# gbbin/DDP-practice

Measured on AMD Instinct MI355X. Metric: images/sec (whole node) + 3-epoch wall-clock, MNIST ConvNet at 1/2/4/8 MI355X, higher is better.
Workload: dtype bf16; 1 GPU; model=ConvNet (2x[Conv5x5-BN-ReLU-MaxPool2] + Linear(1568,10), 29,034 params), global_batch=32, parallelism=dp1, per_rank_batch=32, impl=native (fused HIP kernels, C++ reducer/communicator), sync_bn=False, amp=autocast bf16 + GradScaler, optimizer=SGD(lr=1e-4), hipgraph=True, steps_per_graph=16, comm=none (1 rank), grad_avg=none (1 rank)

## Files before the change

ddp_practice_amd/csrc/kernels/conv5x5.h:

```cpp
#pragma once
#include "convblock_bn.h"

namespace dpa {
namespace cb {

template <int I> struct SH;
template <> struct SH<0> { static constexpr int CIN = 1, COUT = 16, H = 28, W = 28, SPLIT = 4, WROWS = 28; };
template <> struct SH<1> { static constexpr int CIN = 16, COUT = 32, H = 14, W = 14, SPLIT = 2, WROWS = 14; };

__host__ __device__ constexpr int conv5x5_win_rows(int H, int W, int nsplit, bool even) {
  const int HW = H * W, MT = (HW + 15) / 16;
  int mx = 0;
  for (int sp = 0; sp < nsplit; ++sp) {
    const int p0 = 16 * (MT * sp / nsplit), p1e = 16 * (MT * (sp + 1) / nsplit), p1 = p1e < HW ? p1e : HW;
    if (p1 <= p0) return 0;
    int lo = p0 / W - 2, hi = (p1 - 1) / W + 2;
    lo = lo < 0 ? 0 : lo;
    hi = hi > H - 1 ? H - 1 : hi;
    if (even) {
      lo &= ~1;
      hi |= 1;
    }
    mx = hi - lo + 1 > mx ? hi - lo + 1 : mx;
  }
  return mx;
}

template <typename T>
struct BwdEpi {
  const uint8_t* idx;
  const T* xh;
  float* bslab;
};

constexpr int W2F_ROWS = 32, W2F_PITCH = 424;
constexpr int W2D_ROWS = 16, W2D_PITCH = 808;
constexpr int W2F_LEN = W2F_ROWS * W2F_PITCH, W2D_LEN = W2D_ROWS * W2D_PITCH;
template <typename T>
struct WPack {
  const float* w2 = nullptr;
  T* fwd = nullptr;
  T* dgrad = nullptr;
};
template <typename T>
__device__ __forceinline__ void pack_w2(const WPack<T>& pk) {
  const int total = W2F_LEN + W2D_LEN;
  for (int e = blockIdx.x * blockDim.x + threadIdx.x; e < total; e += gridDim.x * blockDim.x) {
    if (e < W2F_LEN) {
      const int co = e / W2F_PITCH, k = e % W2F_PITCH;
      const float v = k < 400 ? pk.w2[(co * 16 + (k & 15)) * 25 + (k >> 4)] : 0.f;
      pk.fwd[e] = Cvt<T>::from_f(v);
    } else {
      const int e2 = e - W2F_LEN;
      const int ci = e2 / W2D_PITCH, k = e2 % W2D_PITCH;
      const float v = k < 800 ? pk.w2[((k & 31) * 16 + ci) * 25 + (24 - (k >> 5))] : 0.f;
      pk.dgrad[e2] = Cvt<T>::from_f(v);
    }
  }
}

struct GatherIn {
  const uint8_t* imgs = nullptr;
  const int64_t* labels = nullptr;
  const int64_t* order = nullptr;
  long long order_len = 0;
  int* ctr = nullptr;
  int64_t* lab_out = nullptr;
  float scale = 1.f, shift = 0.f;
  int nimg = 0;
};

template <typename T, int CIN, int H, int W>
__host__ __device__ constexpr size_t conv5x5_img_bytes() {
  return ((sizeof(T) * (size_t)(H + 4) * (W + 4) * CIN) + 15) / 16 * 16;
}
template <typename T, int CIN, int COUT, int H, int W>
__host__ __device__ constexpr size_t conv5x5_dyn_bytes() {
  return conv5x5_img_bytes<T, CIN, H, W>() + sizeof(T) * (size_t)COUT * (ceil_to(25 * CIN, 32) + 8);
}

template <typename T, int CIN, int COUT, int H, int W, int MODE, int PRO = 0, int EPI = 0, int WPK = 0,
          bool DYN = false, int WR = H>
__device__ __forceinline__ void
conv5x5_body(const T* __restrict__ x, const float* __restrict__ w, const float* __restrict__ bias,
             T* __restrict__ y, float* __restrict__ fslab, float* __restrict__ fstats,
             const float* __restrict__ shift, int nsplit, const PoolIn<T>& pin, const BwdIn<T>& bin,
             const BwdEpi<T>& epi, const T* __restrict__ wpk, const WPack<T>& pk, const int bid,
             const GatherIn& gin = GatherIn{}) {
  static_assert(CIN == 1 || CIN % 8 == 0, "CIN must be 1 or a multiple of 8");
  static_assert(COUT % 16 == 0, "COUT must be a multiple of 16");
  static_assert((H * W) % 4 == 0, "H*W must be a multiple of 4");
  static_assert(PRO != 2 || MODE == 2, "PRO 2 is a data-grad prologue");
  static_assert(PRO != 3 || (CIN == 1 && MODE != 2), "PRO 3 gathers single-channel input images");
  static_assert(EPI == 0 || MODE == 2, "EPI 1 is a data-grad epilogue");
  constexpr int NCH = CIN >= 8 ? CIN / 8 : 1;
  constexpr int HP = H + 4, WPD = W + 4;
  constexpr int K = 25 * CIN;
  constexpr int KP = ceil_to(K, 32);
  constexpr int KS = KP / 32;
  constexpr int KPW = KP + 8;
  constexpr int NT = COUT / 16;
  constexpr int HW = H * W;
  constexpr int MT = (HW + 15) / 16;
  typedef MM<T> mm;

  T* img;
  T* wl;
  if constexpr (DYN) {
    img = reinterpret_cast<T*>(dpa_dyn_lds);
    wl = reinterpret_cast<T*>(dpa_dyn_lds + conv5x5_img_bytes<T, CIN, H, W>());
  } else {
    __shared__ __attribute__((aligned(16))) T img_s[HP * WPD * CIN];
    __shared__ __attribute__((aligned(16))) T wl_s[COUT * KPW];
    img = img_s;
    wl = wl_s;
  }
  constexpr int PPB = NCH <= 16 ? 16 / NCH : 1;
  auto imo = [](int px, int c) -> int {
    if constexpr (NCH <= 1) {
      return px * CIN + c;
    } else {
      return px * CIN + ((((c >> 3) ^ ((px / PPB) & (NCH - 1)))) << 3) + (c & 7);
    }
  };
  __shared__ float lstat[(NTHR / 64) * 2 * COUT];

  const int tid = threadIdx.x;
  const int b = bid / nsplit;
  DPA_STAMP(0);
  const int sp = bid % nsplit;
  const T* xb = x + (size_t)b * CIN * HW;
  const int mt0 = (MT * sp) / nsplit, mt1 = (MT * (sp + 1)) / nsplit;
  constexpr bool WIN = WR < H;
  static_assert(!WIN || PRO == 1 || PRO == 2, "row windows: the BN prologues' staging passes");
  static_assert(WR >= 1 && (PRO != 2 || WR % 2 == 0 || !WIN), "PRO 2 stages whole 2x2 windows");
  constexpr int SR = WIN ? WR : H;
  const int p_lo = mt0 * 16, p_hi = min(mt1 * 16, HW);
  int r_lo = 0, r_n = H, z_lo = 0, z_n = HP;
  if constexpr (WIN) {
    const int oh_lo = p_lo / W, oh_hi = (p_hi - 1) / W;
    r_lo = max(oh_lo - 2, 0);
    int r_hi = min(oh_hi + 2, H - 1);
    if constexpr (PRO == 2) {
      r_lo &= ~1;
      r_hi |= 1;
    }
    r_n = r_hi - r_lo + 1;
    z_lo = oh_lo;
    z_n = oh_hi + 5 - oh_lo;
  }
  float pre_bias[NT], pre_shift[NT];
#pragma unroll
  for (int nt = 0; nt < NT; ++nt) {
    const int co = nt * 16 + (tid & 15);
    pre_bias[nt] = (MODE == 2) ? 0.f : bias[co];
    pre_shift[nt] = (MODE == 0) ? shift[co] : 0.f;
  }

  const T zero = Cvt<T>::from_f(0.f);
  constexpr int WN16 = WPK == 1 ? COUT * KPW * (int)sizeof(T) / 16 : 1;
  constexpr int WIT = (WN16 + NTHR - 1) / NTHR;
  auto load_wpk = [&]() {
    if constexpr (WPK == 1) {
      static_assert((COUT * KPW * sizeof(T)) % 16 == 0, "packed weight tile must be whole 16-B chunks");
      static_assert(COUT * KPW == (MODE == 2 ? W2D_LEN : W2F_LEN), "pre-packed weights exist for layer 2 only");
      typedef __attribute__((address_space(3))) void* lds_ptr_t;
      const uint4* src = reinterpret_cast<const uint4*>(wpk);
      uint4* dstl = reinterpret_cast<uint4*>(wl);
      const int wv0 = (tid >> 6) * 64, ln = tid & 63;
#pragma unroll
      for (int i = 0; i < WIT; ++i) {
        const int c0 = i * NTHR + wv0;
        if (c0 + ln < WN16)
          __builtin_amdgcn_global_load_lds(src + c0 + ln, (lds_ptr_t)(dstl + c0), 16, 0, 0);
      }
    }
  };
  if constexpr (WPK == 1) {
    if constexpr (PRO == 0 || PRO == 3) load_wpk();
  } else {
    if constexpr (KP > K) {
      for (int e = tid; e < COUT * (KP - K); e += NTHR) wl[(e / (KP - K)) * KPW + K + e % (KP - K)] = zero;
    }
    constexpr int KO = 25 * (MODE == 2 ? COUT : CIN);
    stage_f32<COUT * K>(w, [&](int e, float v) {
      const int o = e / KO, rem = e % KO;
      const int i = rem / 25, tap = rem % 25;
      if (MODE == 2)
        wl[i * KPW + (24 - tap) * CIN + o] = Cvt<T>::from_f(v);
      else
        wl[o * KPW + tap * CIN + i] = Cvt<T>::from_f(v);
    });
  }
  if constexpr (WPK == 2) pack_w2<T>(pk);
  DPA_STAMP(1);
  if constexpr ((CIN * sizeof(T)) % 16 == 0) {
    constexpr int G = CIN * (int)sizeof(T) / 16;
    uint4* img4 = reinterpret_cast<uint4*>(img);
    if constexpr (WIN) {
      uint4* row4 = img4 + z_lo * WPD * G;
      for (int e = tid; e < z_n * WPD * G; e += NTHR) {
        const int px = e / G, hp = z_lo + px / WPD, wp = px % WPD;
        if (hp < 2 || hp >= H + 2 || wp < 2 || wp >= W + 2) row4[e] = make_uint4(0u, 0u, 0u, 0u);
      }
    } else {
      for (int e = tid; e < HP * WPD * G; e += NTHR) {
        const int px = e / G, hp = px / WPD, wp = px % WPD;
        if (hp < 2 || hp >= H + 2 || wp < 2 || wp >= W + 2) img4[e] = make_uint4(0u, 0u, 0u, 0u);
      }
    }
  } else {
    static_assert(!WIN, "row windows: whole 16-B channel groups per pixel");
    for (int e = tid; e < HP * WPD * CIN; e += NTHR) {
      const int hp = e / (WPD * CIN), rem = e % (WPD * CIN);
      const int wp = rem / CIN;
      if (hp < 2 || hp >= H + 2 || wp < 2 || wp >= W + 2) img[e] = zero;
    }
  }
  constexpr int EPIX = EPI ? MT * 16 : 1;
  __shared__ uint8_t eidx[EPI ? COUT * EPIX : 1];
  __shared__ T exh[EPI ? COUT * EPIX : 1];
  const int ep0 = mt0 * 16, enp = min(mt1 * 16, HW) - ep0;
  constexpr int EIT = EPI ? (COUT * EPIX + NTHR - 1) / NTHR : 1;
  uint8_t ei[EIT];
  T ex[EIT];
  auto load_epi = [&]() {
    if constexpr (EPI == 1) {
#pragma unroll
      for (int i = 0; i < EIT; ++i) {
        const int e = tid + i * NTHR;
        const int ec = e < COUT * enp ? e : 0;
        const int co = ec / enp, pp = ec % enp;
        const size_t o = ((size_t)b * COUT + co) * HW + ep0 + pp;
        ei[i] = epi.idx[o];
        ex[i] = epi.xh[o];
      }
    }
  };
  auto store_epi = [&]() {
    if constexpr (EPI == 1) {
#pragma unroll
      for (int i = 0; i < EIT; ++i) {
        const int e = tid + i * NTHR;
        if (e < COUT * enp) {
          const int co = e / enp, pp = e % enp;
          eidx[co * EPIX + pp] = ei[i];
          exh[co * EPIX + pp] = ex[i];
        }
      }
    }
  };
  if constexpr (PRO != 2) {
    load_epi();
    store_epi();
  }
  DPA_STAMP(2);
  constexpr int DQ = PRO != 1 ? 1
                     : (CIN % 8 == 0 && sizeof(T) == 2) ? 8 * ((CIN / 8 * SR * W + NTHR - 1) / NTHR)
                                                          : (CIN * SR * W + NTHR - 1) / NTHR;
  int dq_e[DQ];
  T dq_p[DQ], dq_x[DQ];
  uint8_t dq_i[DQ];
#pragma unroll
  for (int d = 0; d < DQ; ++d) dq_e[d] = -1;
  if constexpr (PRO == 0) {
    stage_chw<T, CIN, H, W>(xb, [&](int ci, int h, int ww, T a, T bb) {
      img[imo((h + 2) * WPD + (ww + 2), ci)] = a;
      img[imo((h + 2) * WPD + (ww + 3), ci)] = bb;
    });
  } else if constexpr (PRO == 3) {
    static_assert(HW % 4 == 0 && W % 4 == 0, "4-pixel groups stay inside a row");
    constexpr int G4 = HW / 4, GIT = (G4 + NTHR - 1) / NTHR;
    const int step = __builtin_amdgcn_readfirstlane(*reinterpret_cast<volatile int*>(gin.ctr));
    long long pos = (long long)step * gin.nimg + b;
    pos = pos < gin.order_len ? pos : gin.order_len - 1;
    const int64_t src = gin.order[pos];
    const uint32_t* s4 = reinterpret_cast<const uint32_t*>(gin.imgs + src * HW);
    uint32_t v4[GIT];
#pragma unroll
    for (int i = 0; i < GIT; ++i)
      if (tid + i * NTHR < G4) v4[i] = s4[tid + i * NTHR];
    if (sp == 0 && tid == 0) gin.lab_out[b] = gin.labels[src];
    T* xo = const_cast<T*>(xb);
#pragma unroll
    for (int i = 0; i < GIT; ++i) {
      const int g = tid + i * NTHR;
      if (g < G4) {
        const int h = (4 * g) / W, ww = (4 * g) % W;
        T px[4];
#pragma unroll
        for (int k = 0; k < 4; ++k) {
          px[k] = Cvt<T>::from_f((float)((v4[i] >> (8 * k)) & 0xffu) * gin.scale + gin.shift);
          img[imo((h + 2) * WPD + (ww + k + 2), 0)] = px[k];
        }
        if (sp == 0) {
#pragma unroll
          for (int k = 0; k < 4; ++k) xo[4 * g + k] = px[k];
        }
      }
    }
    if (tid == 0) {
      const int arrived = __hip_atomic_fetch_add(&gin.ctr[1], 1, __ATOMIC_RELAXED, __HIP_MEMORY_SCOPE_AGENT);
      if (arrived == gin.nimg * nsplit - 1) {
        __hip_atomic_store(&gin.ctr[1], 0, __ATOMIC_RELAXED, __HIP_MEMORY_SCOPE_AGENT);
        __hip_atomic_store(&gin.ctr[0], step + 1, __ATOMIC_RELAXED, __HIP_MEMORY_SCOPE_AGENT);
      }
    }
  } else if constexpr (PRO == 1) {
    __shared__ float sc_s[CIN], beta_s[CIN], mean_s[CIN], istd_s[CIN];
    __shared__ float part[NTHR];
    typedef typename Pair2<T>::type P;
    constexpr int RP = SR * W;
    const T* yb = pin.y + (size_t)b * CIN * 4 * HW;
    const bool wr = pin.p_out != nullptr;
    if constexpr (CIN % 8 == 0 && sizeof(T) == 2) {
      constexpr int NO = CIN / 8, NPI = NO * RP, IT8 = (NPI + NTHR - 1) / NTHR;
      P top[IT8][8], bot[IT8][8];
      auto ld8 = [&](int i, int o, int ho, int wo) {
#pragma unroll
        for (int j = 0; j < 8; ++j) {
          const P* src = reinterpret_cast<const P*>(yb + ((size_t)(8 * o + j) * 2 * H + 2 * ho) * 2 * W + 2 * wo);
          top[i][j] = src[0];
          bot[i][j] = src[W];
        }
      };
#pragma unroll
      for (int i = 0; i < IT8; ++i) {
        const int e8 = tid + i * NTHR;
        if constexpr (WIN) {
          const int ec = min(e8, NPI - 1);
          ld8(i, ec / RP, min(r_lo + (ec % RP) / W, H - 1), ec % W);
        } else if (e8 < NPI) {
          ld8(i, e8 / RP, (e8 % RP) / W, e8 % W);
        }
      }
      load_wpk();
      bn_finalize<CIN>(pin.bn, sc_s, beta_s, mean_s, istd_s, part, bid);
      DPA_STAMP(3);
#pragma unroll
      for (int i = 0; i < IT8; ++i) {
        const int e8 = tid + i * NTHR;
        const int o = e8 / RP, hl = (e8 % RP) / W, ho = r_lo + hl, wo = e8 % W;
        if (e8 < NPI && (!WIN || hl < r_n)) {
          const int pix = ho * W + wo;
          const bool own = wr && pix >= p_lo && pix < p_hi;
          unsigned pk[4];
#pragma unroll
          for (int j = 0; j < 8; ++j) {
            const int ci = 8 * o + j;
            float best, xh;
            int bi;
            bn_relu_max4x<T>(top[i][j], bot[i][j], sc_s[ci], beta_s[ci], mean_s[ci], istd_s[ci], best, bi, xh);
            const T pvj = Cvt<T>::from_f(best);
            const unsigned bits = __builtin_bit_cast(unsigned short, pvj);
            if (j & 1) pk[j >> 1] |= bits << 16; else pk[j >> 1] = bits;
            const int e = ci * HW + pix;
            const int d = i * 8 + j;
            dq_e[d] = own ? e : -1;
            dq_p[d] = pvj;
            dq_i[d] = (uint8_t)(bi | (best > 0.f ? IDX_RELU : 0));
            dq_x[d] = Cvt<T>::from_f(xh);
          }
          *reinterpret_cast<uint4*>(&img[imo((ho + 2) * WPD + (wo + 2), 8 * o)]) = make_uint4(pk[0], pk[1], pk[2], pk[3]);
        }
      }
    } else {
      constexpr int NPS = CIN * RP, IT = (NPS + NTHR - 1) / NTHR;
      P top[IT], bot[IT];
      auto ld1 = [&](int i, int ci, int ho, int wo) {
        const P* src = reinterpret_cast<const P*>(yb + ((size_t)ci * 2 * H + 2 * ho) * 2 * W + 2 * wo);
        top[i] = src[0];
        bot[i] = src[W];
      };
#pragma unroll
      for (int i = 0; i < IT; ++i) {
        const int e = tid + i * NTHR;
        if constexpr (WIN) {
          const int ec = min(e, NPS - 1);
          ld1(i, ec / RP, min(r_lo + (ec % RP) / W, H - 1), ec % W);
        } else if (e < NPS) {
          ld1(i, e / RP, (e % RP) / W, e % W);
        }
      }
      load_wpk();
      bn_finalize<CIN>(pin.bn, sc_s, beta_s, mean_s, istd_s, part, bid);
      DPA_STAMP(3);
#pragma unroll
      for (int i = 0; i < IT; ++i) {
        const int e = tid + i * NTHR;
        const int ci = e / RP, hl = (e % RP) / W, ho = r_lo + hl, wo = e % W;
        if (e < NPS && (!WIN || hl < r_n)) {
          const int pix = ho * W + wo;
          float best, xh;
          int bi;
          bn_relu_max4x<T>(top[i], bot[i], sc_s[ci], beta_s[ci], mean_s[ci], istd_s[ci], best, bi, xh);
          const T pv = Cvt<T>::from_f(best);
          img[imo((ho + 2) * WPD + (wo + 2), ci)] = pv;
          dq_e[i] = wr && pix >= p_lo && pix < p_hi ? ci * HW + pix : -1;
          dq_p[i] = pv;
          dq_i[i] = (uint8_t)(bi | (best > 0.f ? IDX_RELU : 0));
          dq_x[i] = Cvt<T>::from_f(xh);
        }
      }
    }
  } else {
    __shared__ float coef[5 * CIN], sums[2 * CIN];
    __shared__ float part[NTHR];
    if constexpr (CIN % 8 == 0 && sizeof(T) == 2) {
      BnBwdStage8<T, CIN, H, W, NTHR, SR> st;
      st.load(bin, b, r_lo);
      DPA_STAMP(8);
      load_wpk();
      bn_bwd_coef<CIN, T>(bin, coef, part, sums, bid);
      load_epi();
      DPA_STAMP(3);
      st.emit(coef, [&](int h, int ww, int c0, uint4 q00, uint4 q01, uint4 q10, uint4 q11) {
        if (WIN && h >= r_n) return;
        const int hp = r_lo + h + 2;
        *reinterpret_cast<uint4*>(&img[imo(hp * WPD + (ww + 2), c0)]) = q00;
        *reinterpret_cast<uint4*>(&img[imo(hp * WPD + (ww + 3), c0)]) = q01;
        *reinterpret_cast<uint4*>(&img[imo((hp + 1) * WPD + (ww + 2), c0)]) = q10;
        *reinterpret_cast<uint4*>(&img[imo((hp + 1) * WPD + (ww + 3), c0)]) = q11;
      });
    } else {
      BnBwdStage<T, CIN, H, W, NTHR, SR> st;
      st.load(bin, b, r_lo);
      DPA_STAMP(8);
      load_wpk();
      bn_bwd_coef<CIN, T>(bin, coef, part, sums, bid);
      load_epi();
      DPA_STAMP(3);
      st.emit(coef, [&](int c, int h, int ww, T v00, T v01, T v10, T v11) {
        if (WIN && h >= r_n) return;
        const int hp = r_lo + h + 2;
        img[imo(hp * WPD + (ww + 2), c)] = v00;
        img[imo(hp * WPD + (ww + 3), c)] = v01;
        img[imo((hp + 1) * WPD + (ww + 2), c)] = v10;
        img[imo((hp + 1) * WPD + (ww + 3), c)] = v11;
      });
    }
    store_epi();
  }
  DPA_STAMP(4);
  __syncthreads();
  DPA_STAMP(5);
  if constexpr (PRO == 1) {
    constexpr int NPO = CIN * HW;
#pragma unroll
    for (int d = 0; d < DQ; ++d)
      if (dq_e[d] >= 0) {
        const size_t o = (size_t)b * NPO + dq_e[d];
        pin.p_out[o] = dq_p[d];
        pin.idx_out[o] = dq_i[d];
        pin.xh_out[o] = dq_x[d];
      }
  }

  const int lane = tid & 63, wv = tid >> 6;
  const int r = lane & 15, q = lane >> 4;

  float s1[NT], s2[NT];
#pragma unroll
  for (int nt = 0; nt < NT; ++nt) s1[nt] = s2[nt] = 0.f;

  for (int mt = mt0 + wv; mt < mt1; mt += NTHR / 64) {
    const int m = mt * 16 + r;
    const int mm_ = m < HW ? m : HW - 1;
    const int oh = mm_ / W, ow = mm_ % W;
    f32x4 acc[NT];
#pragma unroll
    for (int nt = 0; nt < NT; ++nt) acc[nt] = f32x4{0.f, 0.f, 0.f, 0.f};
#pragma unroll
    for (int s = 0; s < KS; ++s) {
      typename mm::frag a;
      if constexpr (CIN == 1) {
#pragma unroll
        for (int j = 0; j < 8; ++j) {
          const int tap = 32 * s + 8 * q + j;
          float v = 0.f;
          if (tap < 25) v = Cvt<T>::to_f(img[(oh + tap / 5) * WPD + ow + tap % 5]);
          a[j] = mm::cv(v);
        }
      } else {
        const int kb = 32 * s + 8 * q;
        int tap = kb / CIN;
        const int ci0 = kb % CIN;
        tap = tap < 25 ? tap : 24;
        a = mm::ld(&img[imo((oh + tap / 5) * WPD + ow + tap % 5, ci0)]);
      }
#pragma unroll
      for (int nt = 0; nt < NT; ++nt) {
        const typename mm::frag bf = mm::ld(&wl[(nt * 16 + r) * KPW + 32 * s + 8 * q]);
        acc[nt] = mm::mma(a, bf, acc[nt]);
      }
    }
    const int pix0 = mt * 16 + 4 * q;
    if (pix0 < HW) {
#pragma unroll
      for (int nt = 0; nt < NT; ++nt) {
        const int co = nt * 16 + r;
        const float bs = pre_bias[nt];
        T* dst = y + ((size_t)b * COUT + co) * HW + pix0;
        const float sh = pre_shift[nt];
#pragma unroll
        for (int i = 0; i < 4; ++i) {
          const float v = acc[nt][i] + bs;
          dst[i] = Cvt<T>::from_f(v);
          if (MODE == 0) {
            const float d = rnd_t<T>(v) - sh;
            s1[nt] += d;
            s2[nt] += d * d;
          }
          if (EPI == 1) {
            const int le = co * EPIX + pix0 - mt0 * 16 + i;
            const float g = (eidx[le] & IDX_RELU) ? rnd_t<T>(v) : 0.f;
            s1[nt] += g;
            s2[nt] += g * Cvt<T>::to_f(exh[le]);
          }
        }
      }
    }
  }
  DPA_STAMP(6);
  if constexpr (MODE == 0 || EPI == 1) {
#pragma unroll
    for (int nt = 0; nt < NT; ++nt) {
      const float a1 = xor32_sum(xor16_sum(s1[nt])), a2 = xor32_sum(xor16_sum(s2[nt]));
      if (q == 0) {
        lstat[wv * 2 * COUT + nt * 16 + r] = a1;
        lstat[wv * 2 * COUT + COUT + nt * 16 + r] = a2;
      }
    }
    __syncthreads();
    float* row = (MODE == 0 ? fslab + (size_t)bid * fslab_row(COUT)
                            : epi.bslab + (size_t)bid * 2 * COUT);
    if (tid < 2 * COUT) {
      float t = 0.f;
#pragma unroll
      for (int w2 = 0; w2 < NTHR / 64; ++w2) t += lstat[w2 * 2 * COUT + tid];
      row[tid] = t;
    }
    if constexpr (MODE == 0) {
      if (tid == 0) {
        const int p0 = mt0 * 16, p1 = min(mt1 * 16, HW);
        row[2 * COUT] = (float)(p1 - p0);
      }
      if (bid == 0 && tid < COUT) fstats[2 * COUT + 1 + tid] = shift[tid];
    }
  }
  DPA_STAMP(7);
}

template <typename T, int CIN, int COUT, int H, int W, int MODE, int PRO = 0, int EPI = 0, int WPK = 0, int WR = H>
__global__ void __launch_bounds__(NTHR)
conv5x5_kernel(const T* __restrict__ x, const float* __restrict__ w, const float* __restrict__ bias,
               T* __restrict__ y, float* __restrict__ fslab, float* __restrict__ fstats,
               const float* __restrict__ shift, int nsplit, PoolIn<T> pin = PoolIn<T>{},
               BwdIn<T> bin = BwdIn<T>{}, BwdEpi<T> epi = BwdEpi<T>{}, const T* __restrict__ wpk = nullptr,
               WPack<T> pk = WPack<T>{}, GatherIn gin = GatherIn{}) {
  conv5x5_body<T, CIN, COUT, H, W, MODE, PRO, EPI, WPK, false, WR>(x, w, bias, y, fslab, fstats, shift, nsplit, pin,
                                                                   bin, epi, wpk, pk, (int)blockIdx.x, gin);
}

}
}
```

ddp_practice_amd/csrc/kernels/convnet_fused.hip:

```cpp
#include <type_traits>

#include "conv5x5.h"
#include "conv5x5_wgrad.h"
#include "comm/xgmi.h"

namespace dpa {
namespace cnf {

using cb::BNParams;
using cb::bn_finalize;
using cb::bn_relu_max4x;
using cb::BwdEpi;
using cb::BwdIn;
using cb::IDX_POS;
using cb::IDX_RELU;
using cb::Pair2;
using cb::PoolIn;
using cb::with_t;

constexpr int HF = 256;
constexpr int NTHR_HB = 256;

template <typename T, int C, int H, int W, int NMAX>
__global__ void __launch_bounds__(HF)
// ... 177 lines not shown
}

typedef std::shared_ptr<xgmi::XgmiComm> XcPtr;
static xgmi::XSite site_of(const XcPtr& xc, int s) { return xc ? xc->site(s) : xgmi::XSite{}; }

int64_t fwd2_split(bool fp32) { return fp32 ? cb::kFwd2SplitT<float> : cb::kFwd2SplitT<__half>; }

template <int NSPLIT, bool EVEN>
constexpr int conv2_wr() {
  constexpr int need = cb::conv5x5_win_rows(14, 14, NSPLIT, EVEN);
  static_assert(need > 0, "conv2: more workgroups per image than 16-pixel tiles");
  return need < 14 ? need : 14;
}
static void conv2_row_window(int wr, int nsplit, bool even, const char* what) {
  const int need = cb::conv5x5_win_rows(14, 14, nsplit, even);
  TORCH_CHECK(need > 0 && (wr >= 14 || need <= wr), what, ": a split in ", nsplit, " stages up to ", need,
              " rows, the kernel's window holds ", wr);
}
template <typename T>
constexpr int kFwd2WR = conv2_wr<cb::kFwd2SplitT<T>, false>();

void conv2_fwd(at::Tensor y1, c10::optional<at::Tensor> fslab1, at::Tensor fstats1, at::Tensor g1, at::Tensor b1,
               at::Tensor rm1, at::Tensor rv1, at::Tensor nbt1, double momentum, double eps, bool train, at::Tensor w2,
               at::Tensor bias2, at::Tensor y2, c10::optional<at::Tensor> fslab2, at::Tensor fstats2, at::Tensor rm2,
               c10::optional<at::Tensor> p1_out, c10::optional<at::Tensor> idx1_out,
               c10::optional<at::Tensor> xh1_out, at::Tensor wpk, XcPtr xc) {
  DPA_CHECK_INPUT(y1); DPA_CHECK_INPUT(w2); DPA_CHECK_INPUT(y2); DPA_CHECK_INPUT(wpk);
  TORCH_CHECK(wpk.numel() == cb::W2F_LEN && wpk.scalar_type() == y1.scalar_type(), "packed conv2 weights");
  const int B = (int)y1.size(0);
  TORCH_CHECK(y1.size(1) == 16 && y1.size(2) == 28 && y1.size(3) == 28 && w2.size(0) == 32 && w2.size(1) == 16,
              "fused conv2 expects the ConvNet shapes");
  TORCH_CHECK(y2.scalar_type() == y1.scalar_type());
  TORCH_CHECK(p1_out.has_value() == idx1_out.has_value() && p1_out.has_value() == xh1_out.has_value());
  if (p1_out.has_value())
    TORCH_CHECK(p1_out->numel() == (int64_t)B * 16 * 196 && idx1_out->numel() == p1_out->numel() &&
                xh1_out->numel() == p1_out->numel());
  const int ns = fwd2_split(y1.scalar_type() == at::kFloat);
  if (train) TORCH_CHECK(fslab2.has_value() && fslab2->numel() == (int64_t)B * ns * cb::fslab_row(32));
  if (B == 0) return;
  BNParams bp = bn_params(fslab1, fstats1, g1, b1, rm1, rv1, nbt1, momentum, eps, train, 16);
  if (train) {
    bp.xs = site_of(xc, xgmi::kSiteFwd1);
    xgmi::set_site_grid(bp.xs, B * ns, "conv2_fwd");
  }
  hipStream_t stream = cur_stream();
  with_t(dt_of(y1), [&](auto tag) {
    typedef decltype(tag) T;
    PoolIn<T> pin{dptr<T>(y1), bp, p1_out.has_value() ? dptr<T>(*p1_out) : nullptr,
                  idx1_out.has_value() ? idx1_out->data_ptr<uint8_t>() : nullptr,
                  xh1_out.has_value() ? dptr<T>(*xh1_out) : nullptr};
    constexpr int WR = kFwd2WR<T>;
    conv2_row_window(WR, ns, false, "conv2_fwd");
    if (train)
      hipLaunchKernelGGL((cb::conv5x5_kernel<T, 16, 32, 14, 14, 0, 1, 0, 1, WR>), dim3(B * ns), dim3(cb::NTHR), 0,
                         stream, nullptr, nullptr, bias2.data_ptr<float>(), dptr<T>(y2), fslab2->data_ptr<float>(),
                         fstats2.data_ptr<float>(), rm2.data_ptr<float>(), ns, pin, BwdIn<T>{}, BwdEpi<T>{},
                         dptr<T>(wpk), cb::WPack<T>{});
    else
      hipLaunchKernelGGL((cb::conv5x5_kernel<T, 16, 32, 14, 14, 1, 1, 0, 1, WR>), dim3(B * ns), dim3(cb::NTHR), 0,
                         stream, nullptr, nullptr, bias2.data_ptr<float>(), dptr<T>(y2), nullptr, nullptr, nullptr,
                         ns, pin, BwdIn<T>{}, BwdEpi<T>{}, dptr<T>(wpk), cb::WPack<T>{});
  });
  DPA_CHECK_LAUNCH();
}

void head_fwd(at::Tensor y2, c10::optional<at::Tensor> fslab2, at::Tensor fstats2, at::Tensor g2, at::Tensor b2,
              at::Tensor rm2, at::Tensor rv2, at::Tensor nbt2, double momentum, double eps, bool train, at::Tensor wfc,
              at::Tensor bfc, at::Tensor logits, c10::optional<at::Tensor> p2_out, c10::optional<at::Tensor> idx2_out,
              c10::optional<at::Tensor> xh2_out, XcPtr xc) {
  DPA_CHECK_INPUT(y2); DPA_CHECK_INPUT(wfc); DPA_CHECK_INPUT(logits);
  const int B = (int)y2.size(0), N = (int)wfc.size(0);
  TORCH_CHECK(y2.size(1) == 32 && y2.size(2) == 14 && y2.size(3) == 14 && wfc.size(1) == 32 * 49,
              "fused head expects the ConvNet shapes");
  TORCH_CHECK(N >= 1 && N <= 64, "fused head supports up to 64 classes");
  TORCH_CHECK(logits.numel() == (int64_t)B * N && logits.scalar_type() == y2.scalar_type());
  TORCH_CHECK(p2_out.has_value() == idx2_out.has_value() && p2_out.has_value() == xh2_out.has_value());
  if (p2_out.has_value())
    TORCH_CHECK(p2_out->numel() == (int64_t)B * 1568 && idx2_out->numel() == p2_out->numel() &&
                xh2_out->numel() == p2_out->numel());
  if (B == 0) return;
  BNParams bp = bn_params(fslab2, fstats2, g2, b2, rm2, rv2, nbt2, momentum, eps, train, 32);
  if (train) {
    bp.xs = site_of(xc, xgmi::kSiteFwd2);
    xgmi::set_site_grid(bp.xs, B, "head_fwd");
    bp.xs.nblk = 0;
  }
  hipStream_t stream = cur_stream();
  with_t(dt_of(y2), [&](auto tag) {
    typedef decltype(tag) T;
    T* po = p2_out.has_value() ? dptr<T>(*p2_out) : nullptr;
    uint8_t* io = idx2_out.has_value() ? idx2_out->data_ptr<uint8_t>() : nullptr;
    T* xo = xh2_out.has_value() ? dptr<T>(*xh2_out) : nullptr;
    auto go = [&](auto nmax) {
      hipLaunchKernelGGL((head_fwd_kernel<T, 32, 14, 14, decltype(nmax)::value>), dim3(B), dim3(HF), 0, stream,
                         dptr<T>(y2), bp, wfc.data_ptr<float>(), bfc.data_ptr<float>(), dptr<T>(logits), po, io, xo,
                         N);
    };
    if (N <= 16) go(std::integral_constant<int, 16>{});
    else go(std::integral_constant<int, 64>{});
  });
  DPA_CHECK_LAUNCH();
}

size_t head_bwd_lds(int64_t B, int64_t N) { return sizeof(float) * (size_t)(B * N + N * 49 + B * 49); }

void head_bwd(at::Tensor dlogits, at::Tensor wfc, at::Tensor p2, at::Tensor idx2, at::Tensor xh2, at::Tensor dwfc,
              at::Tensor dbfc, at::Tensor dgamma2, at::Tensor dbeta2, at::Tensor bsum2, at::Tensor dp2) {
  DPA_CHECK_INPUT(dlogits); DPA_CHECK_INPUT(p2); DPA_CHECK_INPUT(dp2);
  const int B = (int)p2.size(0), N = (int)wfc.size(0);
  TORCH_CHECK(p2.numel() == (int64_t)B * 1568 && dp2.numel() == p2.numel() && xh2.numel() == p2.numel());
  TORCH_CHECK(dlogits.numel() == (int64_t)B * N);
  TORCH_CHECK(dlogits.scalar_type() == p2.scalar_type() && dp2.scalar_type() == p2.scalar_type());
  TORCH_CHECK(bsum2.numel() == 64 && dwfc.numel() == wfc.numel() && dbfc.numel() == N);
  const size_t lds = head_bwd_lds(B, N);
  TORCH_CHECK(lds <= 64 * 1024, "fused head backward: batch too large for LDS (B*N)");
  if (B == 0) return;
  with_t(dt_of(p2), [&](auto tag) {
    typedef decltype(tag) T;
    hipLaunchKernelGGL((head_bwd_kernel<T, 32, 14, 14>), dim3(32), dim3(NTHR_HB), lds, cur_stream(),
                       dptr<T>(dlogits), wfc.data_ptr<float>(), dptr<T>(p2), idx2.data_ptr<uint8_t>(), dptr<T>(xh2), B,
                       N, dwfc.data_ptr<float>(), dbfc.data_ptr<float>(), dgamma2.data_ptr<float>(),
                       dbeta2.data_ptr<float>(), bsum2.data_ptr<float>(), dptr<T>(dp2));
  });
  DPA_CHECK_LAUNCH();
}

static void check_conv1_pack(const at::Tensor& x, const at::Tensor& w1, const at::Tensor& b1, const at::Tensor& y1,
                             const at::Tensor& w2, const at::Tensor& wpk_f, const at::Tensor& wpk_d) {
  const int64_t B = x.size(0);
  TORCH_CHECK(x.size(1) == 1 && x.size(2) == 28 && x.size(3) == 28 && w1.numel() == 16 * 25 && b1.numel() == 16,
              "fused conv1 expects the ConvNet shapes");
  TORCH_CHECK(w2.numel() == 32 * 16 * 25 && w2.scalar_type() == at::kFloat && w1.scalar_type() == at::kFloat);
  TORCH_CHECK(y1.numel() == (int64_t)B * 16 * 784 && y1.scalar_type() == x.scalar_type());
  TORCH_CHECK(wpk_f.numel() == cb::W2F_LEN && wpk_d.numel() == cb::W2D_LEN &&
              wpk_f.scalar_type() == x.scalar_type() && wpk_d.scalar_type() == x.scalar_type());
}

void conv1_fwd_pack(at::Tensor x, at::Tensor w1, at::Tensor b1, at::Tensor y1, c10::optional<at::Tensor> fslab1,
                    c10::optional<at::Tensor> fstats1, c10::optional<at::Tensor> shift1, at::Tensor w2,
                    at::Tensor wpk_f, at::Tensor wpk_d) {
  DPA_CHECK_INPUT(x); DPA_CHECK_INPUT(w1); DPA_CHECK_INPUT(b1); DPA_CHECK_INPUT(y1); DPA_CHECK_INPUT(w2);
  DPA_CHECK_INPUT(wpk_f); DPA_CHECK_INPUT(wpk_d);
  const int B = (int)x.size(0);
  typedef cb::SH<0> S;
  check_conv1_pack(x, w1, b1, y1, w2, wpk_f, wpk_d);
  const bool st = fslab1.has_value();
  if (st)
    TORCH_CHECK(fslab1->numel() == (int64_t)B * S::SPLIT * cb::fslab_row(16) && fstats1->numel() == cb::stats_len(16) &&
                shift1->numel() == 16);
  if (B == 0) return;
  with_t(dt_of(x), [&](auto tag) {
    typedef decltype(tag) T;
    cb::WPack<T> pk{w2.data_ptr<float>(), dptr<T>(wpk_f), dptr<T>(wpk_d)};
    if (st)
      hipLaunchKernelGGL((cb::conv5x5_kernel<T, 1, 16, 28, 28, 0, 0, 0, 2>), dim3(B * S::SPLIT), dim3(cb::NTHR), 0,
                         cur_stream(), dptr<T>(x), w1.data_ptr<float>(), b1.data_ptr<float>(), dptr<T>(y1),
                         fslab1->data_ptr<float>(), fstats1->data_ptr<float>(), shift1->data_ptr<float>(), S::SPLIT,
                         PoolIn<T>{}, BwdIn<T>{}, BwdEpi<T>{}, nullptr, pk);
    else
      hipLaunchKernelGGL((cb::conv5x5_kernel<T, 1, 16, 28, 28, 1, 0, 0, 2>), dim3(B * S::SPLIT), dim3(cb::NTHR), 0,
                         cur_stream(), dptr<T>(x), w1.data_ptr<float>(), b1.data_ptr<float>(), dptr<T>(y1), nullptr,
                         nullptr, nullptr, S::SPLIT, PoolIn<T>{}, BwdIn<T>{}, BwdEpi<T>{}, nullptr, pk);
  });
  DPA_CHECK_LAUNCH();
}

void conv1_fwd_pack_gather(at::Tensor x, at::Tensor w1, at::Tensor b1, at::Tensor y1, at::Tensor fslab1,
                           at::Tensor fstats1, at::Tensor shift1, at::Tensor w2, at::Tensor wpk_f, at::Tensor wpk_d,
                           at::Tensor imgs, at::Tensor labels, at::Tensor order, at::Tensor ctr, at::Tensor lab_out,
                           double scale, double shift) {
  DPA_CHECK_INPUT(x); DPA_CHECK_INPUT(w1); DPA_CHECK_INPUT(b1); DPA_CHECK_INPUT(y1); DPA_CHECK_INPUT(w2);
  DPA_CHECK_INPUT(wpk_f); DPA_CHECK_INPUT(wpk_d); DPA_CHECK_INPUT(imgs); DPA_CHECK_INPUT(labels);
  DPA_CHECK_INPUT(order); DPA_CHECK_INPUT(ctr); DPA_CHECK_INPUT(lab_out);
  const int B = (int)x.size(0);
  typedef cb::SH<0> S;
  TORCH_CHECK(imgs.scalar_type() == at::kByte && imgs.dim() == 3 && imgs.size(1) == 28 && imgs.size(2) == 28,
              "gather: uint8 [N][28][28] dataset");
  TORCH_CHECK(labels.scalar_type() == at::kLong && labels.numel() == imgs.size(0));
  TORCH_CHECK(order.scalar_type() == at::kLong && ctr.scalar_type() == at::kInt && ctr.numel() >= 2);
  TORCH_CHECK(lab_out.scalar_type() == at::kLong && lab_out.numel() == B);
  check_conv1_pack(x, w1, b1, y1, w2, wpk_f, wpk_d);
  TORCH_CHECK(fslab1.numel() == (int64_t)B * S::SPLIT * cb::fslab_row(16) && fstats1.numel() == cb::stats_len(16) &&
              shift1.numel() == 16);
  if (B == 0) return;
  cb::GatherIn gin;
  gin.imgs = imgs.data_ptr<uint8_t>();
  gin.labels = labels.data_ptr<int64_t>();
  gin.order = order.data_ptr<int64_t>();
  gin.order_len = order.numel();
  gin.ctr = ctr.data_ptr<int>();
  gin.lab_out = lab_out.data_ptr<int64_t>();
  gin.scale = (float)scale;
  gin.shift = (float)shift;
  gin.nimg = (int)B;
  with_t(dt_of(x), [&](auto tag) {
    typedef decltype(tag) T;
    cb::WPack<T> pk{w2.data_ptr<float>(), dptr<T>(wpk_f), dptr<T>(wpk_d)};
    hipLaunchKernelGGL((cb::conv5x5_kernel<T, 1, 16, 28, 28, 0, 3, 0, 2>), dim3(B * S::SPLIT), dim3(cb::NTHR), 0,
                       cur_stream(), dptr<T>(x), w1.data_ptr<float>(), b1.data_ptr<float>(), dptr<T>(y1),
                       fslab1.data_ptr<float>(), fstats1.data_ptr<float>(), shift1.data_ptr<float>(), S::SPLIT,
                       PoolIn<T>{}, BwdIn<T>{}, BwdEpi<T>{}, nullptr, pk, gin);
  });
  DPA_CHECK_LAUNCH();
}

#ifndef DPA_DGRAD2_SPLIT
#define DPA_DGRAD2_SPLIT 2
#endif
#ifndef DPA_DGRAD2_SPLIT_F32
#define DPA_DGRAD2_SPLIT_F32 4
#endif
template <typename T>
constexpr int kDgradSplitT = std::is_same<T, float>::value ? DPA_DGRAD2_SPLIT_F32 : DPA_DGRAD2_SPLIT;
static int dgrad_split(bool fp32) { return fp32 ? DPA_DGRAD2_SPLIT_F32 : DPA_DGRAD2_SPLIT; }
template <typename T>
constexpr int kDgrad2WR = conv2_wr<kDgradSplitT<T>, true>();
template <typename T, bool DYN>
__device__ __forceinline__ void conv2_dgrad_role(const T* __restrict__ wpk_d, T* __restrict__ dp1,
                                                 const BwdIn<T>& bi_d, const BwdEpi<T>& ep, int bid) {
  cb::conv5x5_body<T, 32, 16, 14, 14, 2, 2, 1, 1, DYN, kDgrad2WR<T>>(nullptr, nullptr, nullptr, dp1, nullptr, nullptr,
                                                                     nullptr, kDgradSplitT<T>, PoolIn<T>{}, bi_d, ep,
                                                                     wpk_d, cb::WPack<T>{}, bid);
}
int64_t dgrad2_rows(int64_t B, bool fp32) { return B * dgrad_split(fp32); }

void conv2_dgrad(at::Tensor wpk_d, at::Tensor y2, at::Tensor dp2, at::Tensor idx2, at::Tensor fstats2,
                 at::Tensor gsum2, at::Tensor g2, double eps2, at::Tensor dp1, at::Tensor idx1, at::Tensor xh1,
                 at::Tensor bslab1, XcPtr xc) {
  DPA_CHECK_INPUT(y2); DPA_CHECK_INPUT(dp1); DPA_CHECK_INPUT(wpk_d);
  TORCH_CHECK(wpk_d.numel() == cb::W2D_LEN && wpk_d.scalar_type() == y2.scalar_type(),
              "packed conv2 data-grad weights");
  const int B = (int)y2.size(0);
  TORCH_CHECK(y2.size(1) == 32 && y2.size(2) == 14 && dp2.numel() == (int64_t)B * 32 * 49);
  TORCH_CHECK(dp1.numel() == (int64_t)B * 16 * 196 && idx1.numel() == dp1.numel() && xh1.numel() == dp1.numel());
  TORCH_CHECK(bslab1.numel() == dgrad2_rows(B, y2.scalar_type() == at::kFloat) * 32, "BN1 partial-sum slab size");
  if (B == 0) return;
  with_t(dt_of(y2), [&](auto tag) {
    typedef decltype(tag) T;
    constexpr int ds = kDgradSplitT<T>;
    conv2_row_window(kDgrad2WR<T>, ds, true, "conv2_dgrad");
    BwdIn<T> bi = bwd_in<T>(dp2, idx2, y2, fstats2, gsum2, c10::nullopt, g2, eps2, 32, c10::nullopt, c10::nullopt);
    bi.xs = site_of(xc, xgmi::kSiteBwd2Dgrad);
    xgmi::set_site_grid(bi.xs, B * ds, "conv2_dgrad");
    BwdEpi<T> ep{idx1.data_ptr<uint8_t>(), dptr<T>(xh1), bslab1.data_ptr<float>()};
    hipLaunchKernelGGL((cb::conv5x5_kernel<T, 32, 16, 14, 14, 2, 2, 1, 1, kDgrad2WR<T>>), dim3(B * ds), dim3(cb::NTHR),
                       0, cur_stream(), nullptr, nullptr, nullptr, dptr<T>(dp1), nullptr, nullptr, nullptr,
                       ds, PoolIn<T>{}, bi, ep, dptr<T>(wpk_d), cb::WPack<T>{});
  });
  DPA_CHECK_LAUNCH();
}

#ifndef DPA_WG2_NSL
#define DPA_WG2_NSL 2
#endif
constexpr int WG2_NSL = DPA_WG2_NSL;
static_assert(WG2_NSL == 1 || WG2_NSL == 2, "conv2 weight gradient: 1 or 2 input-channel slices");
constexpr int WG1_ROWS_ = 4;
constexpr int WG2_PER_IMG = 2 * WG2_NSL;
int64_t wgrad_bn_rows(int64_t layer, int64_t B);
static int64_t wgrad2_wgs(int64_t B) { return B * WG2_PER_IMG; }

template <typename T, bool DYN>
__device__ __forceinline__ void conv2_wgrad_role(const T* __restrict__ p1, float* __restrict__ wslab2,
                                                 const BwdIn<T>& bi_w, int bid) {
  cb::conv5x5_wgrad_body<T, 16, 32, 14, 14, 14, 2, false, DYN, WG2_NSL>(p1, nullptr, wslab2, WG2_PER_IMG, bi_w, bid);
}
template <typename T>
constexpr size_t conv2_wgrad_lds() {
  return cb::WgradLds<T, 16, 32, 14, 14, 14, WG2_NSL>::bytes;
}
template <typename T>
__global__ void __launch_bounds__(cb::NTHR)
conv2_wgrad_kernel(const T* __restrict__ p1, float* __restrict__ wslab2, BwdIn<T> bi_w) {
  conv2_wgrad_role<T, false>(p1, wslab2, bi_w, (int)blockIdx.x);
}
template <typename T>
struct FcW {
  const T* dls;
  const T* p2;
  float* dw;
  float* db;
  int B = 0, N = 0;
  GradChk chk;
};
constexpr int FC_K = 32 * 49;
constexpr int FC_COLS = cb::NTHR;
constexpr int FC_BMAX = 64, FC_NMAX = 16;
constexpr int FC_BLOCKS = (FC_K + FC_COLS - 1) / FC_COLS;

template <typename T>
__device__ __forceinline__ void fc_wgrad_body(const FcW<T>& f, int wg) {
  __shared__ __attribute__((aligned(16))) float dl_s[FC_BMAX][FC_NMAX];
  const int tid = threadIdx.x;
  const int col = wg * FC_COLS + tid, cc = min(col, FC_K - 1);
  const int B = f.B, N = f.N;
  const bool chk = f.chk.word != nullptr;
  for (int e = tid; e < FC_BMAX * FC_NMAX; e += cb::NTHR) {
    const int b = e / FC_NMAX, n = e % FC_NMAX;
    const float v = Cvt<T>::to_f(f.dls[min(b, B - 1) * N + min(n, N - 1)]);
    dl_s[b][n] = (b < B && n < N) ? v : 0.f;
  }
  float acc[FC_NMAX];
#pragma unroll
  for (int n = 0; n < FC_NMAX; ++n) acc[n] = 0.f;
  __syncthreads();
  for (int b0 = 0; b0 < B; b0 += 32) {
    float pv[32];
#pragma unroll
    for (int u = 0; u < 32; ++u) {
      const int b = b0 + u;
      pv[u] = Cvt<T>::to_f(f.p2[(size_t)min(b, B - 1) * FC_K + cc]) * (b < B ? 1.f : 0.f);
    }
#pragma unroll
    for (int u = 0; u < 32; ++u) {
      const f32x4* row = reinterpret_cast<const f32x4*>(dl_s[min(b0 + u, FC_BMAX - 1)]);
#pragma unroll
      for (int q = 0; q < FC_NMAX / 4; ++q) {
        const f32x4 d = row[q];
        acc[4 * q + 0] += d[0] * pv[u];
        acc[4 * q + 1] += d[1] * pv[u];
        acc[4 * q + 2] += d[2] * pv[u];
        acc[4 * q + 3] += d[3] * pv[u];
      }
    }
  }
  bool bad = false;
  if (col < FC_K) {
#pragma unroll
    for (int n = 0; n < FC_NMAX; ++n)
      if (n < N) {
        f.dw[(size_t)n * FC_K + col] = acc[n];
        bad |= GradChk::bad(acc[n], f.chk.bound);
      }
  }
  if (wg == 0 && tid < N) {
    float a = 0.f;
    for (int b = 0; b < B; ++b) a += dl_s[b][tid];
    f.db[tid] = a;
    bad |= GradChk::bad(a, f.chk.bound);
  }
  if (chk) f.chk.flag(bad);
}

template <typename T>
__global__ void __launch_bounds__(cb::NTHR) fc_wgrad_kernel(FcW<T> f) { fc_wgrad_body<T>(f, (int)blockIdx.x); }

template <typename T>
__global__ void __launch_bounds__(cb::NTHR)
conv2_bwd_kernel(const T* __restrict__ wpk_d, T* __restrict__ dp1, BwdIn<T> bi_d, BwdEpi<T> ep,
                 const T* __restrict__ p1, float* __restrict__ wslab2, BwdIn<T> bi_w, int ndg, int nwg, FcW<T> fw) {
  const int bid = (int)blockIdx.x;
  if (bid < ndg)
    conv2_dgrad_role<T, false>(wpk_d, dp1, bi_d, ep, bid);
  else if (bid < ndg + nwg)
// ... 312 lines not shown
```

Baseline: 790,400 images/s.

## Move layer-2 weight packing to dedicated extra workgroups in the conv1 launch

Layer-2 weight packing (forward and dgrad layouts) used to run as a grid-stride loop inside every conv1 workgroup before the conv work. It now runs in 26 extra workgroups appended to the grid, each with batched loads followed by stores, so conv blocks no longer pay for it. The first-conv path also gets a specialised prologue: one float4 of weights per lane, global loads issued before the LDS zero-fill, gather index and label hoisted with readfirstlane, and the step-counter arrival moved to the kernel end. The cost is extra workgroups and more code-path complexity; moving the counter update to the end also changes when other blocks see the advanced step.

```diff
diff --git a/ddp_practice_amd/csrc/kernels/conv5x5.h b/ddp_practice_amd/csrc/kernels/conv5x5.h
--- a/ddp_practice_amd/csrc/kernels/conv5x5.h
+++ b/ddp_practice_amd/csrc/kernels/conv5x5.h
@@ -36,6 +36,8 @@
 constexpr int W2F_ROWS = 32, W2F_PITCH = 424;
 constexpr int W2D_ROWS = 16, W2D_PITCH = 808;
 constexpr int W2F_LEN = W2F_ROWS * W2F_PITCH, W2D_LEN = W2D_ROWS * W2D_PITCH;
+constexpr int W2P_WGS = 26, W2P_IT = 4;
+static_assert(W2P_WGS * W2P_IT * NTHR >= W2F_LEN + W2D_LEN, "the pack workgroups cover both packs");
 template <typename T>
 struct WPack {
   const float* w2 = nullptr;
@@ -43,20 +45,38 @@
   T* dgrad = nullptr;
 };
 template <typename T>
-__device__ __forceinline__ void pack_w2(const WPack<T>& pk) {
-  const int total = W2F_LEN + W2D_LEN;
-  for (int e = blockIdx.x * blockDim.x + threadIdx.x; e < total; e += gridDim.x * blockDim.x) {
+__device__ __forceinline__ void pack_w2(const WPack<T>& pk, const int wg) {
+  constexpr int TOTAL = W2F_LEN + W2D_LEN;
+  const int tid = threadIdx.x;
+  DPA_STAMP(0);
+  float v[W2P_IT];
+  bool pad[W2P_IT];
+#pragma unroll
+  for (int i = 0; i < W2P_IT; ++i) {
+    const int e = min((wg * W2P_IT + i) * NTHR + tid, TOTAL - 1);
+    int src;
     if (e < W2F_LEN) {
-      const int co = e / W2F_PITCH, k = e % W2F_PITCH;
-      const float v = k < 400 ? pk.w2[(co * 16 + (k & 15)) * 25 + (k >> 4)] : 0.f;
-      pk.fwd[e] = Cvt<T>::from_f(v);
+      const int co = e / W2F_PITCH, k = e % W2F_PITCH, kk = min(k, 399);
+      pad[i] = k >= 400;
+      src = (co * 16 + (kk & 15)) * 25 + (kk >> 4);
     } else {
       const int e2 = e - W2F_LEN;
-      const int ci = e2 / W2D_PITCH, k = e2 % W2D_PITCH;
-      const float v = k < 800 ? pk.w2[((k & 31) * 16 + ci) * 25 + (24 - (k >> 5))] : 0.f;
-      pk.dgrad[e2] = Cvt<T>::from_f(v);
-    }
-  }
+      const int ci = e2 / W2D_PITCH, k = e2 % W2D_PITCH, kk = min(k, 799);
+      pad[i] = k >= 800;
+      src = ((kk & 31) * 16 + ci) * 25 + (24 - (kk >> 5));
+    }
+    v[i] = pk.w2[src];
+  }
+#pragma unroll
+  for (int i = 0; i < W2P_IT; ++i) {
+    const int e = (wg * W2P_IT + i) * NTHR + tid;
+    const T o = Cvt<T>::from_f(pad[i] ? 0.f : v[i]);
+    if (e < W2F_LEN)
+      pk.fwd[e] = o;
+    else if (e < TOTAL)
+      pk.dgrad[e - W2F_LEN] = o;
+  }
+  DPA_STAMP(7);
 }
 
 struct GatherIn {
@@ -128,6 +148,11 @@
   const int tid = threadIdx.x;
   const int b = bid / nsplit;
   DPA_STAMP(0);
+  constexpr bool C1 = WPK == 2;
+  static_assert(!C1 || (CIN == 1 && MODE != 2 && EPI == 0 && (PRO == 0 || PRO == 3)), "WPK 2: the first conv");
+  static_assert(PRO != 3 || C1, "the gather prologue belongs to the fused step's first conv");
+  int step = 0, step_v = 0;
+  if constexpr (PRO == 3) step_v = __hip_atomic_load(gin.ctr, __ATOMIC_RELAXED, __HIP_MEMORY_SCOPE_AGENT);
   const int sp = bid % nsplit;
   const T* xb = x + (size_t)b * CIN * HW;
   const int mt0 = (MT * sp) / nsplit, mt1 = (MT * (sp + 1)) / nsplit;
@@ -178,7 +203,7 @@
   };
   if constexpr (WPK == 1) {
     if constexpr (PRO == 0 || PRO == 3) load_wpk();
-  } else {
+  } else if constexpr (!C1) {
     if constexpr (KP > K) {
       for (int e = tid; e < COUT * (KP - K); e += NTHR) wl[(e / (KP - K)) * KPW + K + e % (KP - K)] = zero;
     }
@@ -192,9 +217,9 @@
         wl[o * KPW + tap * CIN + i] = Cvt<T>::from_f(v);
     });
   }
-  if constexpr (WPK == 2) pack_w2<T>(pk);
   DPA_STAMP(1);
-  if constexpr ((CIN * sizeof(T)) % 16 == 0) {
+  if constexpr (C1) {
+  } else if constexpr ((CIN * sizeof(T)) % 16 == 0) {
     constexpr int G = CIN * (int)sizeof(T) / 16;
     uint4* img4 = reinterpret_cast<uint4*>(img);
     if constexpr (WIN) {
@@ -263,49 +288,98 @@
   uint8_t dq_i[DQ];
 #pragma unroll
   for (int d = 0; d < DQ; ++d) dq_e[d] = -1;
-  if constexpr (PRO == 0) {
+  if constexpr (C1) {
+    constexpr int WN4 = COUT * K / 4;
+    static_assert((COUT * K) % 4 == 0 && WN4 <= NTHR, "one float4 of the weights per lane");
+    const f32x4 w4 = reinterpret_cast<const f32x4*>(w)[min(tid, WN4 - 1)];
+    auto fill_lds = [&]() {
+      for (int e = tid; e < COUT * (KP - K); e += NTHR) wl[(e / (KP - K)) * KPW + K + e % (KP - K)] = zero;
+      for (int e = tid; e < HP * WPD; e += NTHR) {
+        const int hp = e / WPD, wp = e % WPD;
+        if (hp < 2 || hp >= H + 2 || wp < 2 || wp >= W + 2) img[e] = zero;
+      }
+      if (tid < WN4) {
+#pragma unroll
+        for (int j = 0; j < 4; ++j) {
+          const int e = 4 * tid + j;
+          wl[(e / 25) * KPW + e % 25] = Cvt<T>::from_f(w4[j]);
+        }
+      }
+    };
+    if constexpr (PRO == 0) {
+      typedef typename Pair2<T>::type P;
+      static_assert(W % 2 == 0, "pixel pairs stay inside a row");
+      constexpr int NP = HW / 2, XIT = (NP + NTHR - 1) / NTHR;
+      const P* s2 = reinterpret_cast<const P*>(xb);
+      P xv[XIT];
+#pragma unroll
+      for (int i = 0; i < XIT; ++i) xv[i] = s2[min(tid + i * NTHR, NP - 1)];
+      fill_lds();
+      DPA_STAMP(3);
+#pragma unroll
+      for (int i = 0; i < XIT; ++i) {
+        const int e = tid + i * NTHR;
+        if (e < NP) {
+          const int h = (2 * e) / W, ww = (2 * e) % W;
+          T a, bb;
+          __builtin_memcpy(&a, &xv[i], sizeof(T));
+          __builtin_memcpy(&bb, reinterpret_cast<const char*>(&xv[i]) + sizeof(T), sizeof(T));
+          img[imo((h + 2) * WPD + (ww + 2), 0)] = a;
+          img[imo((h + 2) * WPD + (ww + 3), 0)] = bb;
+        }
+      }
+    } else {
+      static_assert(HW % 4 == 0 && W % 4 == 0, "4-pixel groups stay inside a row");
+      constexpr int G4 = HW / 4, GIT = (G4 + NTHR - 1) / NTHR;
+      step = __builtin_amdgcn_readfirstlane(step_v);
+      DPA_STAMP(8);
+      long long pos = (long long)step * gin.nimg + b;
+      pos = pos < gin.order_len ? pos : gin.order_len - 1;
+      const int64_t src_v = gin.order[pos];
+      fill_lds();
+      DPA_STAMP(3);
+      const uint32_t src_lo = __builtin_amdgcn_readfirstlane((uint32_t)src_v);
+      const uint32_t src_hi = __builtin_amdgcn_readfirstlane((uint32_t)((uint64_t)src_v >> 32));
+      const int64_t src = (int64_t)(((uint64_t)src_hi << 32) | src_lo);
+      DPA_STAMP(9);
+      const uint32_t* s4 = reinterpret_cast<const uint32_t*>(gin.imgs + src * HW);
+      uint32_t v4[GIT];
+#pragma unroll
+      for (int i = 0; i < GIT; ++i) v4[i] = s4[min(tid + i * NTHR, G4 - 1)];
+      const int64_t lab_v = gin.labels[src];
+      T px[GIT][4];
+#pragma unroll
+      for (int i = 0; i < GIT; ++i) {
+        const int g = tid + i * NTHR;
+        const int h = (4 * g) / W, ww = (4 * g) % W;
+#pragma unroll
+        for (int k = 0; k < 4; ++k) {
+          px[i][k] = Cvt<T>::from_f((float)((v4[i] >> (8 * k)) & 0xffu) * gin.scale + gin.shift);
+          if (g < G4) img[imo((h + 2) * WPD + (ww + k + 2), 0)] = px[i][k];
+        }
+      }
+      const uint32_t lab_lo = __builtin_amdgcn_readfirstlane((uint32_t)lab_v);
+      const uint32_t lab_hi = __builtin_amdgcn_readfirstlane((uint32_t)((uint64_t)lab_v >> 32));
+      const int64_t lab = (int64_t)(((uint64_t)lab_hi << 32) | lab_lo);
+      DPA_STAMP(10);
+      if (sp == 0) {
+        T* xo = const_cast<T*>(xb);
+#pragma unroll
+        for (int i = 0; i < GIT; ++i) {
+          const int g = tid + i * NTHR;
+          if (g < G4) {
+#pragma unroll
+            for (int k = 0; k < 4; ++k) xo[4 * g + k] = px[i][k];
+          }
+        }
+        if (tid == 0) gin.lab_out[b] = lab;
+      }
+    }
+  } else if constexpr (PRO == 0) {
     stage_chw<T, CIN, H, W>(xb, [&](int ci, int h, int ww, T a, T bb) {
       img[imo((h + 2) * WPD + (ww + 2), ci)] = a;
       img[imo((h + 2) * WPD + (ww + 3), ci)] = bb;
     });
-  } else if constexpr (PRO == 3) {
-    static_assert(HW % 4 == 0 && W % 4 == 0, "4-pixel groups stay inside a row");
-    constexpr int G4 = HW / 4, GIT = (G4 + NTHR - 1) / NTHR;
-    const int step = __builtin_amdgcn_readfirstlane(*reinterpret_cast<volatile int*>(gin.ctr));
-    long long pos = (long long)step * gin.nimg + b;
-    pos = pos < gin.order_len ? pos : gin.order_len - 1;
-    const int64_t src = gin.order[pos];
-    const uint32_t* s4 = reinterpret_cast<const uint32_t*>(gin.imgs + src * HW);
-    uint32_t v4[GIT];
-#pragma unroll
-    for (int i = 0; i < GIT; ++i)
-      if (tid + i * NTHR < G4) v4[i] = s4[tid + i * NTHR];
-    if (sp == 0 && tid == 0) gin.lab_out[b] = gin.labels[src];
-    T* xo = const_cast<T*>(xb);
-#pragma unroll
-    for (int i = 0; i < GIT; ++i) {
-      const int g = tid + i * NTHR;
-      if (g < G4) {
-        const int h = (4 * g) / W, ww = (4 * g) % W;
-        T px[4];
-#pragma unroll
-        for (int k = 0; k < 4; ++k) {
-          px[k] = Cvt<T>::from_f((float)((v4[i] >> (8 * k)) & 0xffu) * gin.scale + gin.shift);
-          img[imo((h + 2) * WPD + (ww + k + 2), 0)] = px[k];
-        }
-        if (sp == 0) {
-#pragma unroll
-          for (int k = 0; k < 4; ++k) xo[4 * g + k] = px[k];
-        }
-      }
-    }
-    if (tid == 0) {
-      const int arrived = __hip_atomic_fetch_add(&gin.ctr[1], 1, __ATOMIC_RELAXED, __HIP_MEMORY_SCOPE_AGENT);
-      if (arrived == gin.nimg * nsplit - 1) {
-        __hip_atomic_store(&gin.ctr[1], 0, __ATOMIC_RELAXED, __HIP_MEMORY_SCOPE_AGENT);
-        __hip_atomic_store(&gin.ctr[0], step + 1, __ATOMIC_RELAXED, __HIP_MEMORY_SCOPE_AGENT);
-      }
-    }
   } else if constexpr (PRO == 1) {
     __shared__ float sc_s[CIN], beta_s[CIN], mean_s[CIN], istd_s[CIN];
     __shared__ float part[NTHR];
@@ -548,6 +622,15 @@
       if (bid == 0 && tid < COUT) fstats[2 * COUT + 1 + tid] = shift[tid];
     }
   }
+  if constexpr (PRO == 3) {
+    if (tid == 0) {
+      const int arrived = __hip_atomic_fetch_add(&gin.ctr[1], 1, __ATOMIC_RELAXED, __HIP_MEMORY_SCOPE_AGENT);
+      if (arrived == gin.nimg * nsplit - 1) {
+        __hip_atomic_store(&gin.ctr[1], 0, __ATOMIC_RELAXED, __HIP_MEMORY_SCOPE_AGENT);
+        __hip_atomic_store(&gin.ctr[0], step + 1, __ATOMIC_RELAXED, __HIP_MEMORY_SCOPE_AGENT);
+      }
+    }
+  }
   DPA_STAMP(7);
 }
 
@@ -558,6 +641,13 @@
                const float* __restrict__ shift, int nsplit, PoolIn<T> pin = PoolIn<T>{},
                BwdIn<T> bin = BwdIn<T>{}, BwdEpi<T> epi = BwdEpi<T>{}, const T* __restrict__ wpk = nullptr,
                WPack<T> pk = WPack<T>{}, GatherIn gin = GatherIn{}) {
+  if constexpr (WPK == 2) {
+    const int nconv = gin.nimg * nsplit;
+    if ((int)blockIdx.x >= nconv) {
+      pack_w2<T>(pk, (int)blockIdx.x - nconv);
+      return;
+    }
+  }
   conv5x5_body<T, CIN, COUT, H, W, MODE, PRO, EPI, WPK, false, WR>(x, w, bias, y, fslab, fstats, shift, nsplit, pin,
                                                                    bin, epi, wpk, pk, (int)blockIdx.x, gin);
 }
diff --git a/ddp_practice_amd/csrc/kernels/convnet_fused.hip b/ddp_practice_amd/csrc/kernels/convnet_fused.hip
--- a/ddp_practice_amd/csrc/kernels/convnet_fused.hip
+++ b/ddp_practice_amd/csrc/kernels/convnet_fused.hip
@@ -353,15 +353,18 @@
   with_t(dt_of(x), [&](auto tag) {
     typedef decltype(tag) T;
     cb::WPack<T> pk{w2.data_ptr<float>(), dptr<T>(wpk_f), dptr<T>(wpk_d)};
+    cb::GatherIn gin;
+    gin.nimg = B;
     if (st)
-      hipLaunchKernelGGL((cb::conv5x5_kernel<T, 1, 16, 28, 28, 0, 0, 0, 2>), dim3(B * S::SPLIT), dim3(cb::NTHR), 0,
-                         cur_stream(), dptr<T>(x), w1.data_ptr<float>(), b1.data_ptr<float>(), dptr<T>(y1),
-                         fslab1->data_ptr<float>(), fstats1->data_ptr<float>(), shift1->data_ptr<float>(), S::SPLIT,
-                         PoolIn<T>{}, BwdIn<T>{}, BwdEpi<T>{}, nullptr, pk);
+      hipLaunchKernelGGL((cb::conv5x5_kernel<T, 1, 16, 28, 28, 0, 0, 0, 2>), dim3(B * S::SPLIT + cb::W2P_WGS),
+                         dim3(cb::NTHR), 0, cur_stream(), dptr<T>(x), w1.data_ptr<float>(), b1.data_ptr<float>(),
+                         dptr<T>(y1), fslab1->data_ptr<float>(), fstats1->data_ptr<float>(),
+                         shift1->data_ptr<float>(), S::SPLIT, PoolIn<T>{}, BwdIn<T>{}, BwdEpi<T>{}, nullptr, pk, gin);
     else
-      hipLaunchKernelGGL((cb::conv5x5_kernel<T, 1, 16, 28, 28, 1, 0, 0, 2>), dim3(B * S::SPLIT), dim3(cb::NTHR), 0,
-                         cur_stream(), dptr<T>(x), w1.data_ptr<float>(), b1.data_ptr<float>(), dptr<T>(y1), nullptr,
-                         nullptr, nullptr, S::SPLIT, PoolIn<T>{}, BwdIn<T>{}, BwdEpi<T>{}, nullptr, pk);
+      hipLaunchKernelGGL((cb::conv5x5_kernel<T, 1, 16, 28, 28, 1, 0, 0, 2>), dim3(B * S::SPLIT + cb::W2P_WGS),
+                         dim3(cb::NTHR), 0, cur_stream(), dptr<T>(x), w1.data_ptr<float>(), b1.data_ptr<float>(),
+                         dptr<T>(y1), nullptr, nullptr, nullptr, S::SPLIT, PoolIn<T>{}, BwdIn<T>{}, BwdEpi<T>{},
+                         nullptr, pk, gin);
   });
   DPA_CHECK_LAUNCH();
 }
@@ -397,10 +400,10 @@
   with_t(dt_of(x), [&](auto tag) {
     typedef decltype(tag) T;
     cb::WPack<T> pk{w2.data_ptr<float>(), dptr<T>(wpk_f), dptr<T>(wpk_d)};
-    hipLaunchKernelGGL((cb::conv5x5_kernel<T, 1, 16, 28, 28, 0, 3, 0, 2>), dim3(B * S::SPLIT), dim3(cb::NTHR), 0,
-                       cur_stream(), dptr<T>(x), w1.data_ptr<float>(), b1.data_ptr<float>(), dptr<T>(y1),
-                       fslab1.data_ptr<float>(), fstats1.data_ptr<float>(), shift1.data_ptr<float>(), S::SPLIT,
-                       PoolIn<T>{}, BwdIn<T>{}, BwdEpi<T>{}, nullptr, pk, gin);
+    hipLaunchKernelGGL((cb::conv5x5_kernel<T, 1, 16, 28, 28, 0, 3, 0, 2>), dim3(B * S::SPLIT + cb::W2P_WGS),
+                       dim3(cb::NTHR), 0, cur_stream(), dptr<T>(x), w1.data_ptr<float>(), b1.data_ptr<float>(),
+                       dptr<T>(y1), fslab1.data_ptr<float>(), fstats1.data_ptr<float>(), shift1.data_ptr<float>(),
+                       S::SPLIT, PoolIn<T>{}, BwdIn<T>{}, BwdEpi<T>{}, nullptr, pk, gin);
   });
   DPA_CHECK_LAUNCH();
 }
```

Measured after the change: 807,100 images/s, median of 6. +2.1%, better.
